# AVianEco/Softspoken

Measured on AMD Instinct MI355X. Metric: audio-seconds processed/sec (whole node), 16 kHz mono, higher is better.
Workload: dtype f16x2

## Files before the change

softspoken_amd/build.py:

```python
from __future__ import annotations

import os
import subprocess
import sys

HERE = os.path.dirname(os.path.abspath(__file__))
CSRC = os.path.join(HERE, "csrc")
OBJ = os.path.join(CSRC, "_obj")
LIB = os.path.join(HERE, "libsoftspoken_hip.so")
DEV_LIB = os.path.join(HERE, "libsoftspoken_hip_dev.so")
SOURCES = ["conv2.hip", "conv2_ups.hip", "conv4.hip", "conv4_ups.hip", "conv1s.hip", "conv9s.hip", "conv9a.hip", "frontend.hip", "heads.hip", "weights.hip", "engine.hip", "host.hip", "abi.hip", "stream.hip", "separate.hip"]
HEADERS = [os.path.join(CSRC, h) for h in ("kernels.h", "engine.h", "dsp.h", "mfma_util.h", "conv4_forms.h", "stream16.h", "net.h", "bands.h", "hostdefs.h", "stream_desc.h", "stream_plan.h")] + [os.path.join(os.path.dirname(HERE), "include", "softspoken.h")]
FLAGS = ["-O3", "--offload-arch=gfx950", "-fPIC", "-std=c++17", "-Wno-unused-value"]
EXTRA_FLAGS = {"frontend.hip": ["-fno-slp-vectorize"], "conv4.hip": ["-fno-slp-vectorize"], "conv4_ups.hip": ["-fno-slp-vectorize"],
               "conv1s.hip": ["-fno-slp-vectorize"], "conv9s.hip": ["-fno-slp-vectorize"], "conv9a.hip": ["-fno-slp-vectorize"]}
DEV_SOURCES = ("conv2.hip", "conv2_ups.hip", "conv4.hip", "conv4_ups.hip", "conv1s.hip", "frontend.hip", "engine.hip", "weights.hip", "abi.hip", "separate.hip")
JITTER_LIB = DEV_LIB


def _hipcc():
    for cand in (os.environ.get("HIPCC"), "/opt/rocm/bin/hipcc"):
        if cand and os.path.exists(cand):
            return cand
    return "hipcc"


def _stale(target, deps):
    if not os.path.exists(target):
        return True
    t = os.path.getmtime(target)
    return any(os.path.getmtime(d) > t for d in deps)


def build(force: bool = False, verbose: bool = True, dev: bool = False, jitter: bool = False) -> str:
    dev = dev or jitter
    os.makedirs(OBJ, exist_ok=True)
    hipcc = _hipcc()
    objs, procs = [], []
    lib = DEV_LIB if dev else LIB
    for src in SOURCES:
        s = os.path.join(CSRC, src)
        d = dev and src in DEV_SOURCES
        o = os.path.join(OBJ, src.replace(".hip", "_dev.o" if d else ".o"))
        objs.append(o)
        if force or _stale(o, [s] + HEADERS):
            cmd = [hipcc] + FLAGS + EXTRA_FLAGS.get(src, []) + (["-DSS_DEVBUILD"] if d else []) + ["-c", s, "-o", o]
            if verbose:
                print("[build]", " ".join(cmd), flush=True)
            procs.append((cmd, subprocess.Popen(cmd, stdout=subprocess.PIPE, stderr=subprocess.STDOUT, text=True)))
    for cmd, p in procs:
        out, _ = p.communicate()
        if p.returncode != 0:
            raise RuntimeError("hipcc failed: %s\n%s" % (" ".join(cmd), out))
    if force or procs or _stale(lib, objs):
        cmd = [hipcc, "--offload-arch=gfx950", "-shared", "-fPIC", "-o", lib] + objs
        if verbose:
            print("[build]", " ".join(cmd), flush=True)
        r = subprocess.run(cmd, stdout=subprocess.PIPE, stderr=subprocess.STDOUT, text=True)
        if r.returncode != 0:
            raise RuntimeError("link failed:\n" + r.stdout)
    return lib


if __name__ == "__main__":
    print(build(force="--force" in sys.argv, dev="--dev" in sys.argv or "--jitter" in sys.argv))
```

softspoken_amd/csrc/conv9a.hip:

```cpp
#include "kernels.h"
#include "stream16.h"
#include <algorithm>
#include <type_traits>

namespace ss {

static constexpr int kUpsFrag = 2 * 2 * 4 * 2 * 2 * 1024;
static constexpr uint32_t kRowB = kW * 64, kRowB8 = (kW / 2) * 64;

struct A9Row8 { u32x4 f[2]; u32x4 h[2]; };

__global__ __launch_bounds__(64 * kS1Waves) __attribute__((amdgpu_waves_per_eu(2, 2)))
void conv3x3_ups_stream16_kernel(ConvArgs a, int rows_per_unit, int total_units) {
    extern __shared__ __attribute__((aligned(16))) char smem[];
    char* sW = smem;
    char* sU = smem + 2 * kBank;

    const int tid = threadIdx.x, lane = tid & 63, wave = __builtin_amdgcn_readfirstlane(tid >> 6);
    const int g = lane >> 4, c = lane & 15;
    for (int p = tid; p < 2 * kBank / 16; p += 64 * kS1Waves) *(u32x4*)(sW + p * 16) = *(const u32x4*)((const char*)a.wpk + (size_t)p * 16);
    for (int p = tid; p < kUpsFrag / 16; p += 64 * kS1Waves) *(u32x4*)(sU + p * 16) = *(const u32x4*)((const char*)a.wpk_b + (size_t)p * 16);
    const f32x4 bias[2] = {*(const f32x4*)(a.bias + 8 * g), *(const f32x4*)(a.bias + 8 * g + 4)};
    __syncthreads();

    const char* wl_base = sW + lane * 16;
    const char* ul_base = sU + lane * 16;
    const int bands = kH / rows_per_unit;
    const int64_t lo = a.lo_delta;
    uint32_t ovf = 0;

    for (int unit = (int)blockIdx.x * kS1Waves + wave; unit < total_units; unit += (int)gridDim.x * kS1Waves) {
        const int s = unit % kStrips32, b = (unit / kStrips32) % bands, n = unit / (kStrips32 * bands);
        const int x0 = 32 * s, y0 = b * rows_per_unit, ylast = y0 + rows_per_unit - 1;
        const uint32_t voff[2] = {(uint32_t)(x0 + 2 * c) * 64u + (uint32_t)g * 16u, (uint32_t)(x0 + 2 * c + 1) * 64u + (uint32_t)g * 16u};
        const uint32_t hoff = (uint32_t)(c < 8 ? max(x0 - 1, 0) : min(x0 + 32, kW - 1)) * 64u + (uint32_t)g * 16u;
        const uint32_t voff8 = (uint32_t)(x0 / 2 + c) * 64u + (uint32_t)g * 16u;
        const uint32_t hoff8 = (uint32_t)(c < 8 ? max(x0 / 2 - 1, 0) : min(x0 / 2 + 16, kW / 2 - 1)) * 64u + (uint32_t)g * 16u;
        const uint32_t hkeep = (c < 8 ? s > 0 : s < kStrips32 - 1) ? 0xffffffffu : 0u;
        const char* c1w = (const char*)a.src0 + (size_t)n * kH * kRowB;
        const char* c8w = (const char*)a.src1 + (size_t)n * (kH / 2) * kRowB8;
        char* ow = (char*)a.out + (size_t)n * kH * kRowB;

        auto load_row = [&](S16RowH& H, int r) {
            const char* p = c1w + (size_t)min(max(r, 0), kH - 1) * kRowB;
#pragma unroll
            for (int t = 0; t < 2; ++t) { H.f[t][0] = *(const u32x4*)(p + voff[t]); H.f[t][1] = *(const u32x4*)(p + lo + voff[t]); }
            H.h[0] = *(const u32x4*)(p + hoff); H.h[1] = *(const u32x4*)(p + lo + hoff);
        };
        auto mask_row = [&](S16RowH& H, int r) {
            const uint32_t rk = (unsigned)r < (unsigned)kH ? 0xffffffffu : 0u;
#pragma unroll
            for (int pq = 0; pq < 2; ++pq)
#pragma unroll
                for (int e = 0; e < 4; ++e) { H.f[0][pq][e] &= rk; H.f[1][pq][e] &= rk; H.h[pq][e] &= hkeep & rk; }
        };
        auto load_row8 = [&](A9Row8& K, int r8) {
            const char* p = c8w + (size_t)min(max(r8, 0), kH / 2 - 1) * kRowB8;
            K.f[0] = *(const u32x4*)(p + voff8); K.f[1] = *(const u32x4*)(p + lo + voff8);
            K.h[0] = *(const u32x4*)(p + hoff8); K.h[1] = *(const u32x4*)(p + lo + hoff8);
        };
        auto mask_row8 = [&](A9Row8& K, int r8) {
            const uint32_t rk = (unsigned)r8 < (unsigned)(kH / 2) ? 0xffffffffu : 0u;
#pragma unroll
            for (int pq = 0; pq < 2; ++pq)
#pragma unroll
                for (int e = 0; e < 4; ++e) { K.f[pq][e] &= rk; K.h[pq][e] &= hkeep & rk; }
        };
        S16RowH H0, H1, H2;
        A9Row8 K0, K1, K2;
        S16Ring3 ring;
        uint32_t ovt = 0;

        auto row_step = [&](auto parity, int y, S16RowH& Ha, const S16RowH& Hb, S16RowH& Hn, A9Row8& Ka, const A9Row8& Kb, A9Row8& Kc) {
            constexpr int par = decltype(parity)::value;
            auto form = [](int q) { return ((q & 1) << 1) | ((q >> 1) & 1); };
            auto rd_set8 = [&](int q) {
                const char* p = ul_base + (((par * 2 + (q >> 2)) * 4 + form(q)) * 4) * 1024;
                ring.rd((q + 1) % 3, p, p + 1024, 2048);
            };
            f32x4 P[2][2];
#pragma unroll
            for (int t = 0; t < 2; ++t)
#pragma unroll
                for (int u = 0; u < 2; ++u) P[t][u] = bias[u];
            s16_taps_shifted(ring, wl_base, Ha, Hb, Hn, P, [&] { rd_set8(0); rd_set8(1); }, [&](int tap) {
                if (tap == 2) load_row(Ha, min(y + 2, ylast + 1));
                if (tap == 5) { mask_row(Hn, y + 1); if constexpr (par != 0) mask_row8(Kc, (y >> 1) + 1); }
            });
#pragma unroll
            for (int q = 0; q < 8; ++q) {
                const int ty = q >> 2, f = form(q), t = f >> 1, slot = (q + 1) % 3;
                const A9Row8& K = par == 0 ? (ty == 0 ? Ka : Kb) : (ty == 0 ? Kb : Kc);
                if (q + 2 < 8) rd_set8(q + 2);
                else if (q == 6) ring.rd_tap(0, wl_base, 0);
                u32x4 B[2];
#pragma unroll
                for (int pq = 0; pq < 2; ++pq) B[pq] = f == 0 ? s16_shr1_halo(K.f[pq], K.h[pq]) : (f == 3 ? s16_shl1_halo(K.f[pq], K.h[pq]) : K.f[pq]);
                __builtin_amdgcn_sched_barrier(0);
                s16_products(ring, slot, B, P[t]);
                __builtin_amdgcn_sched_barrier(0);
                if (par == 0 && q == 3) load_row8(Ka, min((y >> 1) + 2, (ylast >> 1) + 1));
            }
            char* p = ow + (size_t)y * kRowB;
#pragma unroll
            for (int t = 0; t < 2; ++t) {
                float v[2][4];
#pragma unroll
                for (int u = 0; u < 2; ++u)
#pragma unroll
                    for (int r = 0; r < 4; ++r) v[u][r] = relu_i(P[t][u][r]);
                uint32_t kh[4], kl[4];
                s16_split_px(v, kh, kl);
#pragma unroll
                for (int i = 0; i < 4; ++i) ovt = pk_max_u16(ovt, kh[i]);
                *(u32x4*)(p + voff[t]) = u32x4{kh[0], kh[1], kh[2], kh[3]};
                *(u32x4*)(p + lo + voff[t]) = u32x4{kl[0], kl[1], kl[2], kl[3]};
            }
        };

        load_row(H0, y0 - 1); load_row(H1, y0); load_row8(K0, (y0 >> 1) - 1); load_row8(K1, y0 >> 1); load_row(H2, y0 + 1); load_row8(K2, (y0 >> 1) + 1);
        ring.rd_tap(0, wl_base, 0);
        mask_row(H0, y0 - 1); mask_row(H1, y0); mask_row8(K0, (y0 >> 1) - 1); mask_row8(K1, y0 >> 1);
        const std::integral_constant<int, 0> even; const std::integral_constant<int, 1> odd;
        for (int k = 0; k < rows_per_unit; k += 6) {
            row_step(even, y0 + k, H0, H1, H2, K0, K1, K2);
            row_step(odd, y0 + k + 1, H1, H2, H0, K0, K1, K2);
            if (k + 2 >= rows_per_unit) break;
            row_step(even, y0 + k + 2, H2, H0, H1, K1, K2, K0);
            row_step(odd, y0 + k + 3, H0, H1, H2, K1, K2, K0);
            if (k + 4 >= rows_per_unit) break;
            row_step(even, y0 + k + 4, H1, H2, H0, K2, K0, K1);
            row_step(odd, y0 + k + 5, H2, H0, H1, K2, K0, K1);
        }
        ovf = pk_max_u16(ovf, ovt);
    }
    if (((ovf & 0x7fff7fffu) + 0x04000400u) & 0x80008000u) atomicOr(a.range_flag, 1);
}

static bool px64(ActStride s) { return s.pix == 64u; }
bool conv9a_stream_supports(const ConvArgs& a) {
    return a.plain && a.H == kH && a.W == kW && a.Cout == kC && a.C0 == kC && a.C1 == kC && a.src0 && a.src1 && a.wpk && a.wpk_b && a.bias && a.out &&
           !a.pool_out && !a.res_in && !a.res_out && a.lo_delta != 0 && a.range_flag && a.N > 0 && px64(a.s_src0) && px64(a.s_src1) && px64(a.s_out);
}
const char* conv9a_stream_variant() { return "conv3x3_ups_stream16_kernel"; }
size_t conv9a_stream_ups_bytes() { return kUpsFrag; }
bool conv9a_stream_rows_ok(int rows_per_unit) { return rows_per_unit >= 2 && !(rows_per_unit & 1) && kH % rows_per_unit == 0 && rows_per_unit <= kMaxRows; }
double conv9a_stream_issued_macs(int N) { return (double)N * kH * kStrips32 * ((108 + 48) / 3) * (16.0 * 16 * 32); }

hipError_t launch_conv9a_stream(const ConvArgs& a, int rows_per_unit, int grid_override, int num_cus, hipStream_t s) {
    if (!conv9a_stream_supports(a) || !conv9a_stream_rows_ok(rows_per_unit)) return hipErrorInvalidValue;
    const int64_t total = (int64_t)a.N * (kH / rows_per_unit) * kStrips32;
    if (total >= (int64_t)1 << 30) return hipErrorInvalidValue;
    const int cus = num_cus > 0 ? num_cus : 256;
    int grid = (int)std::min<int64_t>(cus, (total + kS1Waves - 1) / kS1Waves);
    if (grid_override > 0) grid = std::min(grid, grid_override);
    static std::atomic<uint64_t> attr_done{0};
    const size_t lds = 2 * (size_t)kBank + kUpsFrag;
    if (hipError_t e = allow_full_lds((const void*)conv3x3_ups_stream16_kernel, attr_done)) return e;
    hipLaunchKernelGGL(conv3x3_ups_stream16_kernel, dim3(grid), dim3(64 * kS1Waves), lds, s, a, rows_per_unit, (int)total);
    return hipGetLastError();
}

}
```

softspoken_amd/csrc/conv9s.hip:

```cpp
#include "kernels.h"
#include "stream16.h"
#include <algorithm>

namespace ss {

static constexpr int kProjFrag = 2 * 2 * 2 * 1024;
static constexpr uint32_t kRowB = kW * 64, kRowB8 = (kW / 2) * 64;

__global__ __launch_bounds__(64 * kS1Waves) __attribute__((amdgpu_waves_per_eu(2, 2)))
void conv9_stream16_kernel(ConvArgs a, int rows_per_unit, int total_units) {
    extern __shared__ __attribute__((aligned(16))) char smem[];
    char* sW = smem;
    char* sP = smem + 2 * kBank;

    const int tid = threadIdx.x, lane = tid & 63, wave = __builtin_amdgcn_readfirstlane(tid >> 6);
    const int g = lane >> 4, c = lane & 15;
    for (int p = tid; p < 2 * kBank / 16; p += 64 * kS1Waves) *(u32x4*)(sW + p * 16) = *(const u32x4*)((const char*)a.wpk + (size_t)p * 16);
    for (int p = tid; p < kProjFrag / 16; p += 64 * kS1Waves) *(u32x4*)(sP + p * 16) = *(const u32x4*)((const char*)a.proj_w + (size_t)p * 16);
    const f32x4 bias[2] = {*(const f32x4*)(a.bias + 8 * g), *(const f32x4*)(a.bias + 8 * g + 4)};
    __syncthreads();

    const char* wl_base = sW + lane * 16;
    const char* pl_base = sP + lane * 16;
    const char* fw_base = (const char*)a.flat_w4 + lane * 16;
    const int bands = kH / rows_per_unit;
    const int64_t lo = a.lo_delta;
    uint32_t ovf = 0;

    for (int unit = (int)blockIdx.x * kS1Waves + wave; unit < total_units; unit += (int)gridDim.x * kS1Waves) {
        const int s = unit % kStrips32, b = (unit / kStrips32) % bands, n = unit / (kStrips32 * bands);
        const int x0 = 32 * s, y0 = b * rows_per_unit, ylast = y0 + rows_per_unit - 1;
        const int xt[2] = {x0 + 2 * c, x0 + 2 * c + 1};
        const uint32_t voff[2] = {(uint32_t)xt[0] * 64u + (uint32_t)g * 16u, (uint32_t)xt[1] * 64u + (uint32_t)g * 16u};
        const uint32_t hoff = (uint32_t)(c < 8 ? max(x0 - 1, 0) : min(x0 + 32, kW - 1)) * 64u + (uint32_t)g * 16u;
        const uint32_t hkeep = (c < 8 ? s > 0 : s < kStrips32 - 1) ? 0xffffffffu : 0u;
        const uint32_t voff8 = (uint32_t)(x0 / 2 + c) * 64u + (uint32_t)g * 16u;
        const char* hw = (const char*)a.src0 + (size_t)n * kH * kRowB;
        const char* c1w = (const char*)a.xp0 + (size_t)n * kH * kRowB;
        const char* c8w = (const char*)a.xp1 + (size_t)n * (kH / 2) * kRowB8;
        char* ow = (char*)a.out + (size_t)n * kH * kRowB;

        auto load_row = [&](S16RowH& H, int r) {
            const char* p = hw + (size_t)min(max(r, 0), kH - 1) * kRowB;
#pragma unroll
            for (int t = 0; t < 2; ++t) { H.f[t][0] = *(const u32x4*)(p + voff[t]); H.f[t][1] = *(const u32x4*)(p + lo + voff[t]); }
            H.h[0] = *(const u32x4*)(p + hoff); H.h[1] = *(const u32x4*)(p + lo + hoff);
        };
        auto mask_row = [&](S16RowH& H, int r) {
            const uint32_t rk = (unsigned)r < (unsigned)kH ? 0xffffffffu : 0u;
#pragma unroll
            for (int pq = 0; pq < 2; ++pq)
#pragma unroll
                for (int e = 0; e < 4; ++e) { H.f[0][pq][e] &= rk; H.f[1][pq][e] &= rk; H.h[pq][e] &= hkeep & rk; }
        };
        S16RowH H0, H1, H2;
        S16Row C1;
        u32x4 C8[2];
        auto load_c1 = [&](int r) {
            const char* p = c1w + (size_t)r * kRowB;
#pragma unroll
            for (int t = 0; t < 2; ++t) { C1.f[t][0] = *(const u32x4*)(p + voff[t]); C1.f[t][1] = *(const u32x4*)(p + lo + voff[t]); }
        };
        auto load_c8 = [&](int r8) {
            const char* p = c8w + (size_t)r8 * kRowB8;
            C8[0] = *(const u32x4*)(p + voff8); C8[1] = *(const u32x4*)(p + lo + voff8);
        };
        f32x4 F[2] = {f32x4{0.f, 0.f, 0.f, 0.f}, f32x4{0.f, 0.f, 0.f, 0.f}};
        uint32_t ovt[2] = {0u, 0u};

        auto row_step = [&](int y, S16RowH& Ha, const S16RowH& Hb, S16RowH& Hn) {
            S16Ring3 ring;
            ring.rd_tap(0, wl_base, 0);
            u32x4 pw[2][2][2];
#pragma unroll
            for (int q = 0; q < 8; ++q) pw[q >> 2][(q >> 1) & 1][q & 1] = *(const u32x4*)(pl_base + q * 1024);
            const u32x4 fwh = *(const u32x4*)(fw_base + (size_t)(2 * y) * 1024), fwl = *(const u32x4*)(fw_base + (size_t)(2 * y + 1) * 1024);
            __builtin_amdgcn_sched_barrier(0);
            f32x4 P[2][2];
#pragma unroll
            for (int t = 0; t < 2; ++t)
#pragma unroll
                for (int u = 0; u < 2; ++u) P[t][u] = bias[u];
#pragma unroll
            for (int src = 0; src < 2; ++src)
#pragma unroll
                for (int pr = 0; pr < 3; ++pr)
#pragma unroll
                    for (int u = 0; u < 2; ++u)
#pragma unroll
                        for (int t = 0; t < 2; ++t) {
                            const int pq = pr == 0 ? 1 : 0;
                            const u32x4& x = src == 0 ? C1.f[t][pq] : C8[pq];
                            P[t][u] = s16_mfma(pw[src][u][pr == 1 ? 1 : 0], x, P[t][u]);
                        }
            __builtin_amdgcn_sched_barrier(0);
            load_c1(min(y + 1, ylast));
            load_c8(min(y + 1, ylast) >> 1);
            __builtin_amdgcn_sched_barrier(0);
            s16_taps_shifted(ring, wl_base, Ha, Hb, Hn, P, [] {}, [&](int tap) {
                if (tap == 2) load_row(Ha, min(y + 2, ylast + 1));
                if (tap == 5) mask_row(Hn, y + 1);
            });
            __builtin_amdgcn_sched_barrier(0);
            float v[2][2][4];
#pragma unroll
            for (int t = 0; t < 2; ++t)
#pragma unroll
                for (int u = 0; u < 2; ++u)
#pragma unroll
                    for (int r = 0; r < 4; ++r) v[t][u][r] = relu_i(P[t][u][r]);
            uint32_t kh[2][4], kl[2][4];
#pragma unroll
            for (int t = 0; t < 2; ++t) {
                s16_split_px(v[t], kh[t], kl[t]);
#pragma unroll
                for (int i = 0; i < 4; ++i) ovt[t] = pk_max_u16(ovt[t], kh[t][i]);
            }
#pragma unroll
            for (int pr = 0; pr < 3; ++pr)
#pragma unroll
                for (int t = 0; t < 2; ++t) {
                    const uint32_t (&k)[4] = pr == 0 ? kl[t] : kh[t];
                    F[t] = s16_mfma(pr == 1 ? fwl : fwh, u32x4{k[0], k[1], k[2], k[3]}, F[t]);
                }
            if (a.store_out) {
                char* p = ow + (size_t)y * kRowB;
#pragma unroll
                for (int t = 0; t < 2; ++t) {
                    *(u32x4*)(p + voff[t]) = u32x4{kh[t][0], kh[t][1], kh[t][2], kh[t][3]};
                    *(u32x4*)(p + lo + voff[t]) = u32x4{kl[t][0], kl[t][1], kl[t][2], kl[t][3]};
                }
            }
        };

        load_row(H0, y0 - 1); load_row(H1, y0); load_c1(y0); load_c8(y0 >> 1); load_row(H2, y0 + 1);
        mask_row(H0, y0 - 1); mask_row(H1, y0);
        int k = 0;
        for (; k + 3 <= rows_per_unit; k += 3) {
            row_step(y0 + k, H0, H1, H2);
            row_step(y0 + k + 1, H1, H2, H0);
            row_step(y0 + k + 2, H2, H0, H1);
        }
        if (k < rows_per_unit) {
            row_step(y0 + k, H0, H1, H2);
            if (k + 1 < rows_per_unit) row_step(y0 + k + 1, H1, H2, H0);
        }
#pragma unroll
        for (int t = 0; t < 2; ++t) {
            if (g == 0) {
                float* fp = a.flat_part + ((size_t)n * bands + b) * 4 * kW + xt[t];
#pragma unroll
                for (int r = 0; r < 4; ++r) fp[r * kW] = F[t][r];
            }
            ovf = pk_max_u16(ovf, ovt[t]);
        }
    }
    if (((ovf & 0x7fff7fffu) + 0x04000400u) & 0x80008000u) atomicOr(a.range_flag, 1);
}

static bool px64(ActStride s) { return s.pix == 64u; }
bool conv9_stream_supports(const ConvArgs& a) {
    return a.H == kH && a.W == kW && a.Cout == kC && a.C0 == kC && a.C1 == 0 && a.C0x == kC && a.C1x == kC && a.src0 && a.xp0 && a.xp1 && a.wpk &&
           a.proj_w && a.bias && a.flat_w4 && a.flat_part && (a.out || !a.store_out) && !a.pool_out && !a.res_in && a.lo_delta != 0 && a.range_flag &&
           a.N > 0 && px64(a.s_src0) && px64(a.s_xp0) && px64(a.s_xp1) && (px64(a.s_out) || !a.store_out);
}
const char* conv9_stream_variant() { return "conv9_stream16_kernel"; }
size_t conv9_stream_proj_bytes() { return kProjFrag; }
size_t conv9_stream_flat_bytes() { return (size_t)kH * 2 * 1024; }
bool conv9_stream_rows_ok(int rows_per_unit) { return rows_per_unit >= 2 && !(rows_per_unit & 1) && kH % rows_per_unit == 0 && rows_per_unit <= kMaxRows; }
int conv9_stream_flat_groups(int rows_per_unit) { return kH / rows_per_unit; }
double conv9_stream_issued_macs(int N) { return (double)N * kH * kStrips32 * ((24 + 108 + 6) / 3) * (16.0 * 16 * 32); }

hipError_t launch_conv9_stream(const ConvArgs& a, int rows_per_unit, int grid_override, int num_cus, hipStream_t s) {
    if (!conv9_stream_supports(a) || !conv9_stream_rows_ok(rows_per_unit)) return hipErrorInvalidValue;
    const int64_t total = (int64_t)a.N * (kH / rows_per_unit) * kStrips32;
    if (total >= (int64_t)1 << 30) return hipErrorInvalidValue;
    const int cus = num_cus > 0 ? num_cus : 256;
    int grid = (int)std::min<int64_t>(cus, (total + kS1Waves - 1) / kS1Waves);
    if (grid_override > 0) grid = std::min(grid, grid_override);
    static std::atomic<uint64_t> attr_done{0};
    const size_t lds = 2 * (size_t)kBank + kProjFrag;
    if (hipError_t e = allow_full_lds((const void*)conv9_stream16_kernel, attr_done)) return e;
    hipLaunchKernelGGL(conv9_stream16_kernel, dim3(grid), dim3(64 * kS1Waves), lds, s, a, rows_per_unit, (int)total);
    return hipGetLastError();
}

}
```

softspoken_amd/csrc/stream16.h:

```cpp
#pragma once
#include "mfma_util.h"

namespace ss {

static constexpr int kH = 128, kW = 256, kC = 32;
static constexpr int kStrips = 9, kStripCols = 30;
static constexpr int kStrips32 = 8;
static constexpr int kBank = 9 * 2 * 1024;
static constexpr int kS1Waves = 8;
static constexpr int kMaxRows = 32;

struct S16Row { u32x4 f[2][2]; };
struct S16RowH { u32x4 f[2][2]; u32x4 h[2]; };
struct S16RowS { u32x4 f[2][2]; u32x4 l[2], r[2]; };

__device__ __forceinline__ f32x4 s16_mfma(const u32x4& a, const u32x4& b, const f32x4& c) {
    return __builtin_amdgcn_mfma_f32_16x16x32_f16(__builtin_bit_cast(f16x8, a), __builtin_bit_cast(f16x8, b), c, 0, 0, 0);
}

__device__ __forceinline__ u32x4 s16_shr1_halo(const u32x4& v, const u32x4& halo) {
    u32x4 r;
#pragma unroll
    for (int e = 0; e < 4; ++e) r[e] = (uint32_t)__builtin_amdgcn_update_dpp((int)halo[e], (int)v[e], 0x111, 0xf, 0xf, false);
    return r;
}
__device__ __forceinline__ u32x4 s16_shl1_halo(const u32x4& v, const u32x4& halo) {
    u32x4 r;
#pragma unroll
    for (int e = 0; e < 4; ++e) r[e] = (uint32_t)__builtin_amdgcn_update_dpp((int)halo[e], (int)v[e], 0x101, 0xf, 0xf, false);
    return r;
}
__device__ __forceinline__ u32x4 s16_operand(const S16RowH& H, int dx, int t, int pq) {
    if (dx == 0) return H.f[t][pq];
    if (dx < 0) return t == 0 ? s16_shr1_halo(H.f[1][pq], H.h[pq]) : H.f[0][pq];
    return t == 0 ? H.f[1][pq] : s16_shl1_halo(H.f[0][pq], H.h[pq]);
}
__device__ __forceinline__ u32x4 s16_operand(const S16RowS& H, int dx, int t, int pq) {
    if (dx == 0) return H.f[t][pq];
    if (dx < 0) return t == 0 ? H.l[pq] : H.f[0][pq];
    return t == 0 ? H.f[1][pq] : H.r[pq];
}
__device__ __forceinline__ void s16_make_shifted(S16RowS& H, const u32x4 (&halo)[2]) {
#pragma unroll
    for (int pq = 0; pq < 2; ++pq) { H.l[pq] = s16_shr1_halo(H.f[1][pq], halo[pq]); H.r[pq] = s16_shl1_halo(H.f[0][pq], halo[pq]); }
}

struct S16Ring3 {
    u32x4 wh[3][2], wl[3][2];
    __device__ __forceinline__ void rd(int slot, const char* hi, const char* lo, int step) {
#pragma unroll
        for (int u = 0; u < 2; ++u) { wh[slot][u] = *(const u32x4*)(hi + u * step); wl[slot][u] = *(const u32x4*)(lo + u * step); }
    }
    __device__ __forceinline__ void rd_tap(int slot, const char* wl_base, int tap) { rd(slot, wl_base + tap * 2048, wl_base + kBank + tap * 2048, 1024); }
};

__device__ __forceinline__ void s16_products(const S16Ring3& ring, int slot, const u32x4 (&B)[2], f32x4 (&Pt)[2]) {
#pragma unroll
    for (int pr = 0; pr < 3; ++pr)
#pragma unroll
        for (int u = 0; u < 2; ++u) Pt[u] = s16_mfma(pr == 1 ? ring.wl[slot][u] : ring.wh[slot][u], B[pr == 0 ? 1 : 0], Pt[u]);
}

template <typename Row, typename Last, typename AfterTap>
__device__ __forceinline__ void s16_taps_shifted(S16Ring3& ring, const char* wl_base, const Row& Ha, const Row& Hb, const Row& Hn,
                                                 f32x4 (&P)[2][2], Last&& before_last, AfterTap&& after_tap) {
#pragma unroll
    for (int tap = 0; tap < 9; ++tap) {
        const int dy = tap / 3, dx = tap % 3 - 1, slot = tap & 1;
        const Row& Hr = dy == 0 ? Ha : (dy == 1 ? Hb : Hn);
        if (tap + 1 < 9) ring.rd_tap(slot ^ 1, wl_base, tap + 1); else before_last();
        u32x4 B[2][2];
#pragma unroll
        for (int pq = 0; pq < 2; ++pq) { B[0][pq] = s16_operand(Hr, dx, 0, pq); B[1][pq] = s16_operand(Hr, dx, 1, pq); }
        __builtin_amdgcn_sched_barrier(0);
#pragma unroll
        for (int pr = 0; pr < 3; ++pr)
#pragma unroll
            for (int u = 0; u < 2; ++u)
#pragma unroll
                for (int t = 0; t < 2; ++t)
                    P[t][u] = s16_mfma(pr == 1 ? ring.wl[slot][u] : ring.wh[slot][u], B[t][pr == 0 ? 1 : 0], P[t][u]);
        __builtin_amdgcn_sched_barrier(0);
        after_tap(tap);
    }
}

__device__ __forceinline__ void s16_split_px(const float (&val)[2][4], uint32_t (&kh)[4], uint32_t (&kl)[4]) {
#pragma unroll
    for (int i = 0; i < 4; ++i) {
        const float e0 = val[i >> 1][2 * (i & 1)], e1 = val[i >> 1][2 * (i & 1) + 1];
        kh[i] = pack_f16(e0, e1);
        kl[i] = split_lo(kh[i], e0, e1);
    }
}

}
```

Baseline: 35030.

## Precompute shifted halo operands once per row in conv9 stream kernels

```diff
diff --git a/softspoken_amd/build.py b/softspoken_amd/build.py
--- a/softspoken_amd/build.py
+++ b/softspoken_amd/build.py
@@ -14,7 +14,7 @@
 FLAGS = ["-O3", "--offload-arch=gfx950", "-fPIC", "-std=c++17", "-Wno-unused-value"]
 EXTRA_FLAGS = {"frontend.hip": ["-fno-slp-vectorize"], "conv4.hip": ["-fno-slp-vectorize"], "conv4_ups.hip": ["-fno-slp-vectorize"],
                "conv1s.hip": ["-fno-slp-vectorize"], "conv9s.hip": ["-fno-slp-vectorize"], "conv9a.hip": ["-fno-slp-vectorize"]}
-DEV_SOURCES = ("conv2.hip", "conv2_ups.hip", "conv4.hip", "conv4_ups.hip", "conv1s.hip", "frontend.hip", "engine.hip", "weights.hip", "abi.hip", "separate.hip")
+DEV_SOURCES = ("conv2.hip", "conv2_ups.hip", "conv4.hip", "conv4_ups.hip", "conv1s.hip", "conv9s.hip", "conv9a.hip", "frontend.hip", "engine.hip", "weights.hip", "abi.hip", "separate.hip")
 JITTER_LIB = DEV_LIB
 
 
diff --git a/softspoken_amd/csrc/conv9a.hip b/softspoken_amd/csrc/conv9a.hip
--- a/softspoken_amd/csrc/conv9a.hip
+++ b/softspoken_amd/csrc/conv9a.hip
@@ -8,10 +8,13 @@
 static constexpr int kUpsFrag = 2 * 2 * 4 * 2 * 2 * 1024;
 static constexpr uint32_t kRowB = kW * 64, kRowB8 = (kW / 2) * 64;
 
-struct A9Row8 { u32x4 f[2]; u32x4 h[2]; };
-
-__global__ __launch_bounds__(64 * kS1Waves) __attribute__((amdgpu_waves_per_eu(2, 2)))
-void conv3x3_ups_stream16_kernel(ConvArgs a, int rows_per_unit, int total_units) {
+struct A9Row8H { u32x4 f[2]; u32x4 h[2]; };
+struct A9Row8 { u32x4 f[2]; u32x4 l[2], r[2]; };
+
+template <S16Ops kOps>
+__device__ __forceinline__ void conv9a_stream16_body(const ConvArgs& a, int rows_per_unit, int total_units) {
+    using Row = std::conditional_t<kOps == kOpsUse, S16RowH, S16RowS>;
+    using Row8 = std::conditional_t<kOps == kOpsUse, A9Row8H, A9Row8>;
     extern __shared__ __attribute__((aligned(16))) char smem[];
     char* sW = smem;
     char* sU = smem + 2 * kBank;
@@ -20,58 +23,104 @@
     const int g = lane >> 4, c = lane & 15;
     for (int p = tid; p < 2 * kBank / 16; p += 64 * kS1Waves) *(u32x4*)(sW + p * 16) = *(const u32x4*)((const char*)a.wpk + (size_t)p * 16);
     for (int p = tid; p < kUpsFrag / 16; p += 64 * kS1Waves) *(u32x4*)(sU + p * 16) = *(const u32x4*)((const char*)a.wpk_b + (size_t)p * 16);
-    const f32x4 bias[2] = {*(const f32x4*)(a.bias + 8 * g), *(const f32x4*)(a.bias + 8 * g + 4)};
+    char* sB = smem + 2 * kBank + kUpsFrag;
+    if (tid < kC) ((float*)sB)[tid] = a.bias[tid];
     __syncthreads();
 
     const char* wl_base = sW + lane * 16;
     const char* ul_base = sU + lane * 16;
+    const char* bl_base = sB + g * 32;
     const int bands = kH / rows_per_unit;
     const int64_t lo = a.lo_delta;
+    const char* c1z[2] = {(const char*)a.src0 - kS16Hdr, (const char*)a.src0 - kS16Hdr + lo};
+    const char* c8z[2] = {(const char*)a.src1 - kS16Hdr, (const char*)a.src1 - kS16Hdr + lo};
+    char* op[2] = {(char*)a.out, (char*)a.out + lo};
+    const uint32_t lv = (uint32_t)c * 128u + (uint32_t)g * 16u, lv8 = (uint32_t)c * 64u + (uint32_t)g * 16u, zoff = kS16Zero + (uint32_t)g * 16u;
+    [[maybe_unused]] const bool has_l = c > 0, has_r = c < 15;
+    const uint32_t lh = (uint32_t)(c < 8 ? -64 : 32 * 64) + (uint32_t)g * 16u, lh8 = (uint32_t)(c < 8 ? -64 : 16 * 64) + (uint32_t)g * 16u;
     uint32_t ovf = 0;
 
     for (int unit = (int)blockIdx.x * kS1Waves + wave; unit < total_units; unit += (int)gridDim.x * kS1Waves) {
         const int s = unit % kStrips32, b = (unit / kStrips32) % bands, n = unit / (kStrips32 * bands);
         const int x0 = 32 * s, y0 = b * rows_per_unit, ylast = y0 + rows_per_unit - 1;
-        const uint32_t voff[2] = {(uint32_t)(x0 + 2 * c) * 64u + (uint32_t)g * 16u, (uint32_t)(x0 + 2 * c + 1) * 64u + (uint32_t)g * 16u};
-        const uint32_t hoff = (uint32_t)(c < 8 ? max(x0 - 1, 0) : min(x0 + 32, kW - 1)) * 64u + (uint32_t)g * 16u;
-        const uint32_t voff8 = (uint32_t)(x0 / 2 + c) * 64u + (uint32_t)g * 16u;
-        const uint32_t hoff8 = (uint32_t)(c < 8 ? max(x0 / 2 - 1, 0) : min(x0 / 2 + 16, kW / 2 - 1)) * 64u + (uint32_t)g * 16u;
-        const uint32_t hkeep = (c < 8 ? s > 0 : s < kStrips32 - 1) ? 0xffffffffu : 0u;
-        const char* c1w = (const char*)a.src0 + (size_t)n * kH * kRowB;
-        const char* c8w = (const char*)a.src1 + (size_t)n * (kH / 2) * kRowB8;
-        char* ow = (char*)a.out + (size_t)n * kH * kRowB;
-
-        auto load_row = [&](S16RowH& H, int r) {
-            const char* p = c1w + (size_t)min(max(r, 0), kH - 1) * kRowB;
-#pragma unroll
-            for (int t = 0; t < 2; ++t) { H.f[t][0] = *(const u32x4*)(p + voff[t]); H.f[t][1] = *(const u32x4*)(p + lo + voff[t]); }
-            H.h[0] = *(const u32x4*)(p + hoff); H.h[1] = *(const u32x4*)(p + lo + hoff);
-        };
-        auto mask_row = [&](S16RowH& H, int r) {
-            const uint32_t rk = (unsigned)r < (unsigned)kH ? 0xffffffffu : 0u;
-#pragma unroll
-            for (int pq = 0; pq < 2; ++pq)
-#pragma unroll
-                for (int e = 0; e < 4; ++e) { H.f[0][pq][e] &= rk; H.f[1][pq][e] &= rk; H.h[pq][e] &= hkeep & rk; }
-        };
-        auto load_row8 = [&](A9Row8& K, int r8) {
-            const char* p = c8w + (size_t)min(max(r8, 0), kH / 2 - 1) * kRowB8;
-            K.f[0] = *(const u32x4*)(p + voff8); K.f[1] = *(const u32x4*)(p + lo + voff8);
-            K.h[0] = *(const u32x4*)(p + hoff8); K.h[1] = *(const u32x4*)(p + lo + hoff8);
-        };
-        auto mask_row8 = [&](A9Row8& K, int r8) {
-            const uint32_t rk = (unsigned)r8 < (unsigned)(kH / 2) ? 0xffffffffu : 0u;
-#pragma unroll
-            for (int pq = 0; pq < 2; ++pq)
-#pragma unroll
-                for (int e = 0; e < 4; ++e) { K.f[pq][e] &= rk; K.h[pq][e] &= hkeep & rk; }
-        };
-        S16RowH H0, H1, H2;
-        A9Row8 K0, K1, K2;
+        [[maybe_unused]] const uint32_t voff[2] = {(uint32_t)(x0 + 2 * c) * 64u + (uint32_t)g * 16u, (uint32_t)(x0 + 2 * c + 1) * 64u + (uint32_t)g * 16u};
+        [[maybe_unused]] const uint32_t hoff = (uint32_t)(c < 8 ? max(x0 - 1, 0) : min(x0 + 32, kW - 1)) * 64u + (uint32_t)g * 16u;
+        [[maybe_unused]] const uint32_t voff8 = (uint32_t)(x0 / 2 + c) * 64u + (uint32_t)g * 16u;
+        [[maybe_unused]] const uint32_t hoff8 = (uint32_t)(c < 8 ? max(x0 / 2 - 1, 0) : min(x0 / 2 + 16, kW / 2 - 1)) * 64u + (uint32_t)g * 16u;
+        [[maybe_unused]] const uint32_t hkeep = (c < 8 ? s > 0 : s < kStrips32 - 1) ? 0xffffffffu : 0u;
+        [[maybe_unused]] const bool keep_l = s > 0 || has_l, keep_r = s < kStrips32 - 1 || has_r;
+        const uint32_t win = (uint32_t)n * (kH * kRowB) + (uint32_t)x0 * 64u, win8 = (uint32_t)n * ((kH / 2) * kRowB8) + (uint32_t)(x0 / 2) * 64u;
+        [[maybe_unused]] const char* c1w = (const char*)a.src0 + (size_t)n * kH * kRowB;
+        [[maybe_unused]] const char* c8w = (const char*)a.src1 + (size_t)n * (kH / 2) * kRowB8;
+
+        auto load_row = [&](Row& H, int r) {
+            const bool in = (unsigned)r < (unsigned)kH;
+            const uint32_t o = kS16Hdr + win + (uint32_t)r * kRowB;
+            if constexpr (kOps == kOpsOnce) {
+                const uint32_t of = in ? o + lv : zoff, oh = in && hkeep ? o + lh : zoff;
+#pragma unroll
+                for (int pq = 0; pq < 2; ++pq) s16_load_halo(H, pq, c1z[pq], of, oh);
+            } else if constexpr (kOps == kOpsLoad) {
+                const uint32_t of = in ? o + lv : zoff, ol = in && keep_l ? o + lv : zoff, orr = in && keep_r ? o + lv : zoff;
+#pragma unroll
+                for (int pq = 0; pq < 2; ++pq) s16_load_shifted(H, pq, c1z[pq], of, ol, orr);
+            } else {
+                const char* p = c1w + (size_t)min(max(r, 0), kH - 1) * kRowB;
+#pragma unroll
+                for (int t = 0; t < 2; ++t) { H.f[t][0] = *(const u32x4*)(p + voff[t]); H.f[t][1] = *(const u32x4*)(p + lo + voff[t]); }
+                H.h[0] = *(const u32x4*)(p + hoff); H.h[1] = *(const u32x4*)(p + lo + hoff);
+            }
+        };
+        auto load_row8 = [&](Row8& K, int r8) {
+            const bool in = (unsigned)r8 < (unsigned)(kH / 2);
+            const uint32_t o = kS16Hdr + win8 + (uint32_t)r8 * kRowB8;
+            if constexpr (kOps == kOpsOnce) {
+                const uint32_t of = in ? o + lv8 : zoff, oh = in && hkeep ? o + lh8 : zoff;
+#pragma unroll
+                for (int pq = 0; pq < 2; ++pq) { K.f[pq] = s16_ld(c8z[pq], of); K.l[pq] = s16_ld(c8z[pq], oh); }
+            } else if constexpr (kOps == kOpsLoad) {
+                const uint32_t of = in ? o + lv8 : zoff, ol = in && keep_l ? o + lv8 : zoff, orr = in && keep_r ? o + lv8 : zoff;
+#pragma unroll
+                for (int pq = 0; pq < 2; ++pq) { K.f[pq] = s16_ld(c8z[pq], of); K.l[pq] = s16_ld(c8z[pq], ol, -64); K.r[pq] = s16_ld(c8z[pq], orr, 64); }
+            } else {
+                const char* p = c8w + (size_t)min(max(r8, 0), kH / 2 - 1) * kRowB8;
+                K.f[0] = *(const u32x4*)(p + voff8); K.f[1] = *(const u32x4*)(p + lo + voff8);
+                K.h[0] = *(const u32x4*)(p + hoff8); K.h[1] = *(const u32x4*)(p + lo + hoff8);
+            }
+        };
+        auto arrived = [&](Row& H, int r) {
+            if constexpr (kOps == kOpsOnce) s16_shift_arrived(H);
+            if constexpr (kOps == kOpsUse) {
+                const uint32_t rk = (unsigned)r < (unsigned)kH ? 0xffffffffu : 0u;
+#pragma unroll
+                for (int pq = 0; pq < 2; ++pq)
+#pragma unroll
+                    for (int e = 0; e < 4; ++e) { H.f[0][pq][e] &= rk; H.f[1][pq][e] &= rk; H.h[pq][e] &= hkeep & rk; }
+            }
+        };
+        auto arrived8 = [&](Row8& K, int r8) {
+            if constexpr (kOps == kOpsOnce) {
+#pragma unroll
+                for (int pq = 0; pq < 2; ++pq) { const u32x4 halo = K.l[pq]; K.l[pq] = s16_shr1_halo(K.f[pq], halo); K.r[pq] = s16_shl1_halo(K.f[pq], halo); }
+            }
+            if constexpr (kOps == kOpsUse) {
+                const uint32_t rk = (unsigned)r8 < (unsigned)(kH / 2) ? 0xffffffffu : 0u;
+#pragma unroll
+                for (int pq = 0; pq < 2; ++pq)
+#pragma unroll
+                    for (int e = 0; e < 4; ++e) { K.f[pq][e] &= rk; K.h[pq][e] &= hkeep & rk; }
+            }
+        };
+        auto operand8 = [&](const Row8& K, int f, int pq) -> u32x4 {
+            if (f == 1 || f == 2) return K.f[pq];
+            if constexpr (kOps != kOpsUse) return f == 0 ? K.l[pq] : K.r[pq];
+            else return f == 0 ? s16_shr1_halo(K.f[pq], K.h[pq]) : s16_shl1_halo(K.f[pq], K.h[pq]);
+        };
+        Row H0, H1, H2;
+        Row8 K0, K1, K2;
         S16Ring3 ring;
-        uint32_t ovt = 0;
-
-        auto row_step = [&](auto parity, int y, S16RowH& Ha, const S16RowH& Hb, S16RowH& Hn, A9Row8& Ka, const A9Row8& Kb, A9Row8& Kc) {
+
+        auto row_step = [&](auto parity, int y, Row& Ha, const Row& Hb, Row& Hn, Row8& Ka, const Row8& Kb, Row8& Kc) {
             constexpr int par = decltype(parity)::value;
             auto form = [](int q) { return ((q & 1) << 1) | ((q >> 1) & 1); };
             auto rd_set8 = [&](int q) {
@@ -82,26 +131,26 @@
 #pragma unroll
             for (int t = 0; t < 2; ++t)
 #pragma unroll
-                for (int u = 0; u < 2; ++u) P[t][u] = bias[u];
+                for (int u = 0; u < 2; ++u) P[t][u] = *(const f32x4*)(bl_base + u * 16);
             s16_taps_shifted(ring, wl_base, Ha, Hb, Hn, P, [&] { rd_set8(0); rd_set8(1); }, [&](int tap) {
                 if (tap == 2) load_row(Ha, min(y + 2, ylast + 1));
-                if (tap == 5) { mask_row(Hn, y + 1); if constexpr (par != 0) mask_row8(Kc, (y >> 1) + 1); }
+                if (tap == 5) { arrived(Hn, y + 1); if constexpr (par != 0) arrived8(Kc, (y >> 1) + 1); }
             });
 #pragma unroll
             for (int q = 0; q < 8; ++q) {
                 const int ty = q >> 2, f = form(q), t = f >> 1, slot = (q + 1) % 3;
-                const A9Row8& K = par == 0 ? (ty == 0 ? Ka : Kb) : (ty == 0 ? Kb : Kc);
+                const Row8& K = par == 0 ? (ty == 0 ? Ka : Kb) : (ty == 0 ? Kb : Kc);
                 if (q + 2 < 8) rd_set8(q + 2);
                 else if (q == 6) ring.rd_tap(0, wl_base, 0);
                 u32x4 B[2];
 #pragma unroll
-                for (int pq = 0; pq < 2; ++pq) B[pq] = f == 0 ? s16_shr1_halo(K.f[pq], K.h[pq]) : (f == 3 ? s16_shl1_halo(K.f[pq], K.h[pq]) : K.f[pq]);
+                for (int pq = 0; pq < 2; ++pq) B[pq] = operand8(K, f, pq);
                 __builtin_amdgcn_sched_barrier(0);
                 s16_products(ring, slot, B, P[t]);
                 __builtin_amdgcn_sched_barrier(0);
                 if (par == 0 && q == 3) load_row8(Ka, min((y >> 1) + 2, (ylast >> 1) + 1));
             }
-            char* p = ow + (size_t)y * kRowB;
+            const uint32_t o = win + (uint32_t)y * kRowB + lv;
 #pragma unroll
             for (int t = 0; t < 2; ++t) {
                 float v[2][4];
@@ -112,15 +161,15 @@
                 uint32_t kh[4], kl[4];
                 s16_split_px(v, kh, kl);
 #pragma unroll
-                for (int i = 0; i < 4; ++i) ovt = pk_max_u16(ovt, kh[i]);
-                *(u32x4*)(p + voff[t]) = u32x4{kh[0], kh[1], kh[2], kh[3]};
-                *(u32x4*)(p + lo + voff[t]) = u32x4{kl[0], kl[1], kl[2], kl[3]};
+                for (int i = 0; i < 4; ++i) ovf = pk_max_u16(ovf, kh[i]);
+                s16_st(op[0], o, 64 * t, u32x4{kh[0], kh[1], kh[2], kh[3]});
+                s16_st(op[1], o, 64 * t, u32x4{kl[0], kl[1], kl[2], kl[3]});
             }
         };
 
         load_row(H0, y0 - 1); load_row(H1, y0); load_row8(K0, (y0 >> 1) - 1); load_row8(K1, y0 >> 1); load_row(H2, y0 + 1); load_row8(K2, (y0 >> 1) + 1);
         ring.rd_tap(0, wl_base, 0);
-        mask_row(H0, y0 - 1); mask_row(H1, y0); mask_row8(K0, (y0 >> 1) - 1); mask_row8(K1, y0 >> 1);
+        arrived(H0, y0 - 1); arrived(H1, y0); arrived8(K0, (y0 >> 1) - 1); arrived8(K1, y0 >> 1);
         const std::integral_constant<int, 0> even; const std::integral_constant<int, 1> odd;
         for (int k = 0; k < rows_per_unit; k += 6) {
             row_step(even, y0 + k, H0, H1, H2, K0, K1, K2);
@@ -132,17 +181,29 @@
             row_step(even, y0 + k + 4, H1, H2, H0, K2, K0, K1);
             row_step(odd, y0 + k + 5, H2, H0, H1, K2, K0, K1);
         }
-        ovf = pk_max_u16(ovf, ovt);
     }
     if (((ovf & 0x7fff7fffu) + 0x04000400u) & 0x80008000u) atomicOr(a.range_flag, 1);
 }
+
+__global__ __launch_bounds__(64 * kS1Waves) __attribute__((amdgpu_waves_per_eu(2, 2)))
+void conv3x3_ups_stream16_kernel(ConvArgs a, int rows_per_unit, int total_units) { conv9a_stream16_body<kOpsOnce>(a, rows_per_unit, total_units); }
+#ifdef SS_DEVBUILD
+__global__ __launch_bounds__(64 * kS1Waves) __attribute__((amdgpu_waves_per_eu(2, 2)))
+void conv3x3_ups_stream16_load_kernel(ConvArgs a, int rows_per_unit, int total_units) { conv9a_stream16_body<kOpsLoad>(a, rows_per_unit, total_units); }
+__global__ __launch_bounds__(64 * kS1Waves) __attribute__((amdgpu_waves_per_eu(2, 2)))
+void conv3x3_ups_stream16_dpp_kernel(ConvArgs a, int rows_per_unit, int total_units) { conv9a_stream16_body<kOpsUse>(a, rows_per_unit, total_units); }
+#endif
 
 static bool px64(ActStride s) { return s.pix == 64u; }
 bool conv9a_stream_supports(const ConvArgs& a) {
     return a.plain && a.H == kH && a.W == kW && a.Cout == kC && a.C0 == kC && a.C1 == kC && a.src0 && a.src1 && a.wpk && a.wpk_b && a.bias && a.out &&
-           !a.pool_out && !a.res_in && !a.res_out && a.lo_delta != 0 && a.range_flag && a.N > 0 && px64(a.s_src0) && px64(a.s_src1) && px64(a.s_out);
-}
-const char* conv9a_stream_variant() { return "conv3x3_ups_stream16_kernel"; }
+           !a.pool_out && !a.res_in && !a.res_out && a.lo_delta != 0 && a.range_flag && a.N > 0 && px64(a.s_src0) && px64(a.s_src1) && px64(a.s_out) &&
+           (uint64_t)a.N * kH * kRowB + kS16Hdr <= 0xffffffffull;
+}
+static int conv9a_stream_ops() { const int o = dev_env("SOFTSPOKEN_C9A_OPS", 0); return o == kOpsLoad || o == kOpsUse ? o : kOpsOnce; }
+const char* conv9a_stream_variant() {
+    return conv9a_stream_ops() == kOpsLoad ? "conv3x3_ups_stream16_load_kernel" : conv9a_stream_ops() == kOpsUse ? "conv3x3_ups_stream16_dpp_kernel" : "conv3x3_ups_stream16_kernel";
+}
 size_t conv9a_stream_ups_bytes() { return kUpsFrag; }
 bool conv9a_stream_rows_ok(int rows_per_unit) { return rows_per_unit >= 2 && !(rows_per_unit & 1) && kH % rows_per_unit == 0 && rows_per_unit <= kMaxRows; }
 double conv9a_stream_issued_macs(int N) { return (double)N * kH * kStrips32 * ((108 + 48) / 3) * (16.0 * 16 * 32); }
@@ -155,9 +216,17 @@
     int grid = (int)std::min<int64_t>(cus, (total + kS1Waves - 1) / kS1Waves);
     if (grid_override > 0) grid = std::min(grid, grid_override);
     static std::atomic<uint64_t> attr_done{0};
-    const size_t lds = 2 * (size_t)kBank + kUpsFrag;
+    const size_t lds = 2 * (size_t)kBank + kUpsFrag + kC * sizeof(float);
+    auto kernel = conv3x3_ups_stream16_kernel;
+#ifdef SS_DEVBUILD
+    static std::atomic<uint64_t> dev_done[3];
+    if (conv9a_stream_ops() != kOpsOnce) {
+        kernel = conv9a_stream_ops() == kOpsLoad ? conv3x3_ups_stream16_load_kernel : conv3x3_ups_stream16_dpp_kernel;
+        if (hipError_t e = allow_full_lds((const void*)kernel, dev_done[conv9a_stream_ops()])) return e;
+    } else
+#endif
     if (hipError_t e = allow_full_lds((const void*)conv3x3_ups_stream16_kernel, attr_done)) return e;
-    hipLaunchKernelGGL(conv3x3_ups_stream16_kernel, dim3(grid), dim3(64 * kS1Waves), lds, s, a, rows_per_unit, (int)total);
+    hipLaunchKernelGGL(kernel, dim3(grid), dim3(64 * kS1Waves), lds, s, a, rows_per_unit, (int)total);
     return hipGetLastError();
 }
 
diff --git a/softspoken_amd/csrc/conv9s.hip b/softspoken_amd/csrc/conv9s.hip
--- a/softspoken_amd/csrc/conv9s.hip
+++ b/softspoken_amd/csrc/conv9s.hip
@@ -1,14 +1,16 @@
 #include "kernels.h"
 #include "stream16.h"
 #include <algorithm>
+#include <type_traits>
 
 namespace ss {
 
 static constexpr int kProjFrag = 2 * 2 * 2 * 1024;
 static constexpr uint32_t kRowB = kW * 64, kRowB8 = (kW / 2) * 64;
 
-__global__ __launch_bounds__(64 * kS1Waves) __attribute__((amdgpu_waves_per_eu(2, 2)))
-void conv9_stream16_kernel(ConvArgs a, int rows_per_unit, int total_units) {
+template <S16Ops kOps>
+__device__ __forceinline__ void conv9_stream16_body(const ConvArgs& a, int rows_per_unit, int total_units) {
+    using Row = std::conditional_t<kOps == kOpsUse, S16RowH, S16RowS>;
     extern __shared__ __attribute__((aligned(16))) char smem[];
     char* sW = smem;
     char* sP = smem + 2 * kBank;
@@ -22,9 +24,14 @@
 
     const char* wl_base = sW + lane * 16;
     const char* pl_base = sP + lane * 16;
-    const char* fw_base = (const char*)a.flat_w4 + lane * 16;
+    const char* fw_base = (const char*)a.flat_w4;
     const int bands = kH / rows_per_unit;
     const int64_t lo = a.lo_delta;
+    const char* hz[2] = {(const char*)a.src0 - kS16Hdr, (const char*)a.src0 - kS16Hdr + lo};
+    const char* c1p[2] = {(const char*)a.xp0, (const char*)a.xp0 + lo};
+    const char* c8p[2] = {(const char*)a.xp1, (const char*)a.xp1 + lo};
+    char* op[2] = {(char*)a.out, (char*)a.out + lo};
+    const uint32_t zoff = kS16Zero + (uint32_t)g * 16u;
     uint32_t ovf = 0;
 
     for (int unit = (int)blockIdx.x * kS1Waves + wave; unit < total_units; unit += (int)gridDim.x * kS1Waves) {
@@ -32,49 +39,64 @@
         const int x0 = 32 * s, y0 = b * rows_per_unit, ylast = y0 + rows_per_unit - 1;
         const int xt[2] = {x0 + 2 * c, x0 + 2 * c + 1};
         const uint32_t voff[2] = {(uint32_t)xt[0] * 64u + (uint32_t)g * 16u, (uint32_t)xt[1] * 64u + (uint32_t)g * 16u};
-        const uint32_t hoff = (uint32_t)(c < 8 ? max(x0 - 1, 0) : min(x0 + 32, kW - 1)) * 64u + (uint32_t)g * 16u;
-        const uint32_t hkeep = (c < 8 ? s > 0 : s < kStrips32 - 1) ? 0xffffffffu : 0u;
+        [[maybe_unused]] const uint32_t hoff = (uint32_t)(c < 8 ? max(x0 - 1, 0) : min(x0 + 32, kW - 1)) * 64u + (uint32_t)g * 16u;
+        [[maybe_unused]] const uint32_t hkeep = (c < 8 ? s > 0 : s < kStrips32 - 1) ? 0xffffffffu : 0u;
+        [[maybe_unused]] const bool keep_l = s > 0 || c > 0, keep_r = s < kStrips32 - 1 || c < 15;
         const uint32_t voff8 = (uint32_t)(x0 / 2 + c) * 64u + (uint32_t)g * 16u;
-        const char* hw = (const char*)a.src0 + (size_t)n * kH * kRowB;
-        const char* c1w = (const char*)a.xp0 + (size_t)n * kH * kRowB;
-        const char* c8w = (const char*)a.xp1 + (size_t)n * (kH / 2) * kRowB8;
-        char* ow = (char*)a.out + (size_t)n * kH * kRowB;
-
-        auto load_row = [&](S16RowH& H, int r) {
-            const char* p = hw + (size_t)min(max(r, 0), kH - 1) * kRowB;
-#pragma unroll
-            for (int t = 0; t < 2; ++t) { H.f[t][0] = *(const u32x4*)(p + voff[t]); H.f[t][1] = *(const u32x4*)(p + lo + voff[t]); }
-            H.h[0] = *(const u32x4*)(p + hoff); H.h[1] = *(const u32x4*)(p + lo + hoff);
-        };
-        auto mask_row = [&](S16RowH& H, int r) {
-            const uint32_t rk = (unsigned)r < (unsigned)kH ? 0xffffffffu : 0u;
-#pragma unroll
-            for (int pq = 0; pq < 2; ++pq)
-#pragma unroll
-                for (int e = 0; e < 4; ++e) { H.f[0][pq][e] &= rk; H.f[1][pq][e] &= rk; H.h[pq][e] &= hkeep & rk; }
-        };
-        S16RowH H0, H1, H2;
+        [[maybe_unused]] const char* hw = (const char*)a.src0 + (size_t)n * kH * kRowB;
+        const uint32_t win = (uint32_t)n * (kH * kRowB), win8 = (uint32_t)n * ((kH / 2) * kRowB8);
+
+        auto load_row = [&](Row& H, int r) {
+            const bool in = (unsigned)r < (unsigned)kH;
+            const uint32_t o = kS16Hdr + win + (uint32_t)r * kRowB;
+            if constexpr (kOps == kOpsOnce) {
+                const uint32_t of = in ? o + voff[0] : zoff, oh = in && hkeep ? o + hoff : zoff;
+#pragma unroll
+                for (int pq = 0; pq < 2; ++pq) s16_load_halo(H, pq, hz[pq], of, oh);
+            } else if constexpr (kOps == kOpsLoad) {
+                const uint32_t of = in ? o + voff[0] : zoff, ol = in && keep_l ? o + voff[0] : zoff, orr = in && keep_r ? o + voff[0] : zoff;
+#pragma unroll
+                for (int pq = 0; pq < 2; ++pq) s16_load_shifted(H, pq, hz[pq], of, ol, orr);
+            } else {
+                const char* p = hw + (size_t)min(max(r, 0), kH - 1) * kRowB;
+#pragma unroll
+                for (int t = 0; t < 2; ++t) { H.f[t][0] = *(const u32x4*)(p + voff[t]); H.f[t][1] = *(const u32x4*)(p + lo + voff[t]); }
+                H.h[0] = *(const u32x4*)(p + hoff); H.h[1] = *(const u32x4*)(p + lo + hoff);
+            }
+        };
+        auto arrived = [&](Row& H, int r) {
+            if constexpr (kOps == kOpsOnce) s16_shift_arrived(H);
+            if constexpr (kOps == kOpsUse) {
+                const uint32_t rk = (unsigned)r < (unsigned)kH ? 0xffffffffu : 0u;
+#pragma unroll
+                for (int pq = 0; pq < 2; ++pq)
+#pragma unroll
+                    for (int e = 0; e < 4; ++e) { H.f[0][pq][e] &= rk; H.f[1][pq][e] &= rk; H.h[pq][e] &= hkeep & rk; }
+            }
+        };
+        Row H0, H1, H2;
         S16Row C1;
         u32x4 C8[2];
         auto load_c1 = [&](int r) {
-            const char* p = c1w + (size_t)r * kRowB;
-#pragma unroll
-            for (int t = 0; t < 2; ++t) { C1.f[t][0] = *(const u32x4*)(p + voff[t]); C1.f[t][1] = *(const u32x4*)(p + lo + voff[t]); }
+            const uint32_t o = win + (uint32_t)r * kRowB + voff[0];
+#pragma unroll
+            for (int t = 0; t < 2; ++t) { C1.f[t][0] = s16_ld(c1p[0], o, 64 * t); C1.f[t][1] = s16_ld(c1p[1], o, 64 * t); }
         };
         auto load_c8 = [&](int r8) {
-            const char* p = c8w + (size_t)r8 * kRowB8;
-            C8[0] = *(const u32x4*)(p + voff8); C8[1] = *(const u32x4*)(p + lo + voff8);
+            const uint32_t o = win8 + (uint32_t)r8 * kRowB8 + voff8;
+            C8[0] = s16_ld(c8p[0], o); C8[1] = s16_ld(c8p[1], o);
         };
         f32x4 F[2] = {f32x4{0.f, 0.f, 0.f, 0.f}, f32x4{0.f, 0.f, 0.f, 0.f}};
         uint32_t ovt[2] = {0u, 0u};
 
-        auto row_step = [&](int y, S16RowH& Ha, const S16RowH& Hb, S16RowH& Hn) {
+        auto row_step = [&](int y, Row& Ha, const Row& Hb, Row& Hn) {
             S16Ring3 ring;
             ring.rd_tap(0, wl_base, 0);
             u32x4 pw[2][2][2];
 #pragma unroll
             for (int q = 0; q < 8; ++q) pw[q >> 2][(q >> 1) & 1][q & 1] = *(const u32x4*)(pl_base + q * 1024);
-            const u32x4 fwh = *(const u32x4*)(fw_base + (size_t)(2 * y) * 1024), fwl = *(const u32x4*)(fw_base + (size_t)(2 * y + 1) * 1024);
+            const uint32_t fo = (uint32_t)y * 2048u + (uint32_t)lane * 16u;
+            const u32x4 fwh = s16_ld(fw_base, fo), fwl = s16_ld(fw_base, fo, 1024);
             __builtin_amdgcn_sched_barrier(0);
             f32x4 P[2][2];
 #pragma unroll
@@ -99,7 +121,7 @@
             __builtin_amdgcn_sched_barrier(0);
             s16_taps_shifted(ring, wl_base, Ha, Hb, Hn, P, [] {}, [&](int tap) {
                 if (tap == 2) load_row(Ha, min(y + 2, ylast + 1));
-                if (tap == 5) mask_row(Hn, y + 1);
+                if (tap == 5) arrived(Hn, y + 1);
             });
             __builtin_amdgcn_sched_barrier(0);
             float v[2][2][4];
@@ -124,17 +146,18 @@
                     F[t] = s16_mfma(pr == 1 ? fwl : fwh, u32x4{k[0], k[1], k[2], k[3]}, F[t]);
                 }
             if (a.store_out) {
-                char* p = ow + (size_t)y * kRowB;
+                uint32_t o = win + (uint32_t)y * kRowB + voff[0];
+                asm volatile("" : "+v"(o));
 #pragma unroll
                 for (int t = 0; t < 2; ++t) {
-                    *(u32x4*)(p + voff[t]) = u32x4{kh[t][0], kh[t][1], kh[t][2], kh[t][3]};
-                    *(u32x4*)(p + lo + voff[t]) = u32x4{kl[t][0], kl[t][1], kl[t][2], kl[t][3]};
+                    s16_st(op[0], o, 64 * t, u32x4{kh[t][0], kh[t][1], kh[t][2], kh[t][3]});
+                    s16_st(op[1], o, 64 * t, u32x4{kl[t][0], kl[t][1], kl[t][2], kl[t][3]});
                 }
             }
         };
 
         load_row(H0, y0 - 1); load_row(H1, y0); load_c1(y0); load_c8(y0 >> 1); load_row(H2, y0 + 1);
-        mask_row(H0, y0 - 1); mask_row(H1, y0);
+        arrived(H0, y0 - 1); arrived(H1, y0);
         int k = 0;
         for (; k + 3 <= rows_per_unit; k += 3) {
             row_step(y0 + k, H0, H1, H2);
@@ -158,13 +181,26 @@
     if (((ovf & 0x7fff7fffu) + 0x04000400u) & 0x80008000u) atomicOr(a.range_flag, 1);
 }
 
+__global__ __launch_bounds__(64 * kS1Waves) __attribute__((amdgpu_waves_per_eu(2, 2)))
+void conv9_stream16_kernel(ConvArgs a, int rows_per_unit, int total_units) { conv9_stream16_body<kOpsOnce>(a, rows_per_unit, total_units); }
+#ifdef SS_DEVBUILD
+__global__ __launch_bounds__(64 * kS1Waves) __attribute__((amdgpu_waves_per_eu(2, 2)))
+void conv9_stream16_load_kernel(ConvArgs a, int rows_per_unit, int total_units) { conv9_stream16_body<kOpsLoad>(a, rows_per_unit, total_units); }
+__global__ __launch_bounds__(64 * kS1Waves) __attribute__((amdgpu_waves_per_eu(2, 2)))
+void conv9_stream16_dpp_kernel(ConvArgs a, int rows_per_unit, int total_units) { conv9_stream16_body<kOpsUse>(a, rows_per_unit, total_units); }
+#endif
+
 static bool px64(ActStride s) { return s.pix == 64u; }
 bool conv9_stream_supports(const ConvArgs& a) {
     return a.H == kH && a.W == kW && a.Cout == kC && a.C0 == kC && a.C1 == 0 && a.C0x == kC && a.C1x == kC && a.src0 && a.xp0 && a.xp1 && a.wpk &&
            a.proj_w && a.bias && a.flat_w4 && a.flat_part && (a.out || !a.store_out) && !a.pool_out && !a.res_in && a.lo_delta != 0 && a.range_flag &&
-           a.N > 0 && px64(a.s_src0) && px64(a.s_xp0) && px64(a.s_xp1) && (px64(a.s_out) || !a.store_out);
-}
-const char* conv9_stream_variant() { return "conv9_stream16_kernel"; }
+           a.N > 0 && px64(a.s_src0) && px64(a.s_xp0) && px64(a.s_xp1) && (px64(a.s_out) || !a.store_out) &&
+           (uint64_t)a.N * kH * kRowB + kS16Hdr <= 0xffffffffull;
+}
+static int conv9_stream_ops() { const int o = dev_env("SOFTSPOKEN_C9S_OPS", 0); return o == kOpsLoad || o == kOpsUse ? o : kOpsOnce; }
+const char* conv9_stream_variant() {
+    return conv9_stream_ops() == kOpsLoad ? "conv9_stream16_load_kernel" : conv9_stream_ops() == kOpsUse ? "conv9_stream16_dpp_kernel" : "conv9_stream16_kernel";
+}
 size_t conv9_stream_proj_bytes() { return kProjFrag; }
 size_t conv9_stream_flat_bytes() { return (size_t)kH * 2 * 1024; }
 bool conv9_stream_rows_ok(int rows_per_unit) { return rows_per_unit >= 2 && !(rows_per_unit & 1) && kH % rows_per_unit == 0 && rows_per_unit <= kMaxRows; }
@@ -180,8 +216,16 @@
     if (grid_override > 0) grid = std::min(grid, grid_override);
     static std::atomic<uint64_t> attr_done{0};
     const size_t lds = 2 * (size_t)kBank + kProjFrag;
+    auto kernel = conv9_stream16_kernel;
+#ifdef SS_DEVBUILD
+    static std::atomic<uint64_t> dev_done[3];
+    if (conv9_stream_ops() != kOpsOnce) {
+        kernel = conv9_stream_ops() == kOpsLoad ? conv9_stream16_load_kernel : conv9_stream16_dpp_kernel;
+        if (hipError_t e = allow_full_lds((const void*)kernel, dev_done[conv9_stream_ops()])) return e;
+    } else
+#endif
     if (hipError_t e = allow_full_lds((const void*)conv9_stream16_kernel, attr_done)) return e;
-    hipLaunchKernelGGL(conv9_stream16_kernel, dim3(grid), dim3(64 * kS1Waves), lds, s, a, rows_per_unit, (int)total);
+    hipLaunchKernelGGL(kernel, dim3(grid), dim3(64 * kS1Waves), lds, s, a, rows_per_unit, (int)total);
     return hipGetLastError();
 }
 
diff --git a/softspoken_amd/csrc/stream16.h b/softspoken_amd/csrc/stream16.h
--- a/softspoken_amd/csrc/stream16.h
+++ b/softspoken_amd/csrc/stream16.h
@@ -43,6 +43,19 @@
 __device__ __forceinline__ void s16_make_shifted(S16RowS& H, const u32x4 (&halo)[2]) {
 #pragma unroll
     for (int pq = 0; pq < 2; ++pq) { H.l[pq] = s16_shr1_halo(H.f[1][pq], halo[pq]); H.r[pq] = s16_shl1_halo(H.f[0][pq], halo[pq]); }
+}
+
+enum S16Ops { kOpsOnce = 0, kOpsLoad = 1, kOpsUse = 2 };
+static constexpr uint32_t kS16Hdr = 256, kS16Zero = 64;
+__device__ __forceinline__ u32x4 s16_ld(const char* base, uint32_t off, int imm = 0) { return *(const u32x4*)(base + (uint64_t)off + (int64_t)imm); }
+__device__ __forceinline__ void s16_st(char* base, uint32_t off, int imm, const u32x4& v) { *(u32x4*)(base + (uint64_t)off + (int64_t)imm) = v; }
+__device__ __forceinline__ void s16_load_halo(S16RowS& H, int pq, const char* base, uint32_t off, uint32_t off_h) {
+    H.f[0][pq] = s16_ld(base, off); H.f[1][pq] = s16_ld(base, off, 64); H.l[pq] = s16_ld(base, off_h);
+}
+__device__ __forceinline__ void s16_shift_arrived(S16RowS& H) { const u32x4 halo[2] = {H.l[0], H.l[1]}; s16_make_shifted(H, halo); }
+__device__ __forceinline__ void s16_load_shifted(S16RowS& H, int pq, const char* base, uint32_t off, uint32_t off_l, uint32_t off_r) {
+    H.f[0][pq] = s16_ld(base, off); H.f[1][pq] = s16_ld(base, off, 64);
+    H.l[pq] = s16_ld(base, off_l, -64); H.r[pq] = s16_ld(base, off_r, 128);
 }
 
 struct S16Ring3 {
```

New measurement: 35360 (median of 6 runs). Within noise of the previous version (+1.0%).
